# stecrotti/MPSKit.jl

Hardware: AMD Instinct MI355X
Metric: DMRG sweeps/sec + ddAC matvec achieved-TFLOP/s, Heisenberg L=100 D=1024 fp64 (higher is better)
Workload: dtype f64; 1 GPU; Heisenberg S=1/2 FiniteMPS L=100 D=1024 d=2 W=5 fp64, 1-site DMRG sweep (2L-2 site updates), fixed Krylov budget 8 matvecs/site; parallelism=single GPU

## Files before the change

mpskit.jl_amd/csrc/mpsk_cholqr.hip:

```cpp
#include <hip/hip_runtime.h>
#include <cmath>
#include <cstdio>
#include <cstdlib>
#include <cstring>
#include <string>
#include "mpsk_internal.h"

namespace mpsk {

constexpr int CB = 64;
constexpr double CQ_FIRSTORDER_MAX = 1.0e-7;

__global__ __launch_bounds__(256) void cq_pad_identity_kernel(double* __restrict__ G, int npad, int n) {
  const int64_t total = (int64_t)npad * npad;
  for (int64_t e = blockIdx.x * (int64_t)blockDim.x + threadIdx.x; e < total; e += (int64_t)gridDim.x * blockDim.x) {
    int r = (int)(e % npad), c = (int)(e / npad);
    if (r >= n || c >= n) G[e] = (r == c) ? 1.0 : 0.0;
  }
}

__global__ __launch_bounds__(256) void cq_shift_kernel(double* __restrict__ G, int npad, int n, double factor) {
  __shared__ double red[4];
  __shared__ double sh;
  double acc = 0.0;
  for (int i = threadIdx.x; i < n; i += 256) acc += G[i + (int64_t)i * npad];
  for (int off = 32; off > 0; off >>= 1) acc += __shfl_down(acc, off, 64);
  if ((threadIdx.x & 63) == 0) red[threadIdx.x >> 6] = acc;
  __syncthreads();
  if (threadIdx.x == 0) sh = factor * (red[0] + red[1] + red[2] + red[3]);
  __syncthreads();
  const double s = sh;
  for (int i = threadIdx.x; i < n; i += 256) G[i + (int64_t)i * npad] += s;
}

typedef double cq_d4 __attribute__((ext_vector_type(4)));

__device__ __forceinline__ double cq_readlane(double v, int lane) {
  int lo = __double2loint(v), hi = __double2hiint(v);
  lo = __builtin_amdgcn_readlane(lo, lane);
  hi = __builtin_amdgcn_readlane(hi, lane);
  return __hiloint2double(hi, lo);
}

__device__ __forceinline__ void piv_rsqrt(double x, double* rs_out, double* sq_out) {
  double r = __builtin_amdgcn_rsq(x);
  r = r * (1.5 - 0.5 * x * r * r);
  r = r * (1.5 - 0.5 * x * r * r);
  double s = x * r;
  s = s + 0.5 * r * (x - s * s);
  *rs_out = r;
  *sq_out = s;
}

constexpr int CQ_SL = 66;
constexpr size_t CQ_STEP_LDS = (size_t)3 * CB * CQ_SL * sizeof(double);

typedef double cq_d2 __attribute__((ext_vector_type(2)));
__device__ __forceinline__ void cq_fetch_tile(cq_d2 (&r)[8], const double* __restrict__ src, int npad, int tid) {
#pragma unroll
  for (int q = 0; q < 8; ++q) {
    const int v = tid + 256 * q, r2 = (v & 31) * 2, c = v >> 5;
    r[q] = *reinterpret_cast<const cq_d2*>(&src[r2 + (int64_t)c * npad]);
  }
}
__device__ __forceinline__ void cq_put_tile(double* __restrict__ dst, const cq_d2 (&r)[8], int tid) {
#pragma unroll
  for (int q = 0; q < 8; ++q) {
    const int v = tid + 256 * q, r2 = (v & 31) * 2, c = v >> 5;
    *reinterpret_cast<cq_d2*>(&dst[c * CQ_SL + r2]) = r[q];
  }
}

__device__ __forceinline__ void cq_prod(cq_d4 (&acc)[2][2], const double* __restrict__ tA, const double* __restrict__ tB,
                                        double sign, int wr, int wc, int fr, int fq) {
  for (int l0 = 0; l0 < CB; l0 += 4) {
    double af[2], bf[2];
#pragma unroll
    for (int ti = 0; ti < 2; ++ti) af[ti] = sign * tA[(32 * wr + 16 * ti + fr) * CQ_SL + l0 + fq];
#pragma unroll
    for (int tj = 0; tj < 2; ++tj) bf[tj] = tB[(32 * wc + 16 * tj + fr) * CQ_SL + l0 + fq];
#pragma unroll
    for (int ti = 0; ti < 2; ++ti)
#pragma unroll
      for (int tj = 0; tj < 2; ++tj)
        acc[ti][tj] = __builtin_amdgcn_mfma_f64_16x16x4f64(af[ti], bf[tj], acc[ti][tj], 0, 0, 0);
  }
}

constexpr int CQ_GS = 16;

__global__ __launch_bounds__(256) void cq_gram_reduce_kernel(const double* __restrict__ Gp, int npad, double* __restrict__ G) {
  const int64_t np2 = (int64_t)npad * npad;
  for (int64_t e = blockIdx.x * (int64_t)blockDim.x + threadIdx.x; e < np2; e += (int64_t)gridDim.x * blockDim.x) {
    const int r = (int)(e % npad), c = (int)(e / npad);
    if (r / CB > c / CB) continue;
    double acc = 0.0;
#pragma unroll
    for (int sp = 0; sp < CQ_GS; ++sp) acc += Gp[(int64_t)sp * np2 + e];
    G[e] = acc;
  }
}

__device__ __forceinline__ void cq_fetch_tile_g(cq_d2 (&r)[8], const double* __restrict__ src, int ld, int row0, int col0,
                                                int m, int n, int tid) {
#pragma unroll
  for (int q = 0; q < 8; ++q) {
    const int v = tid + 256 * q, r2 = (v & 31) * 2, c = v >> 5;
    const int gr = row0 + r2, gc = col0 + c;
    cq_d2 t = {0.0, 0.0};
    if (gc < n) {
      const double* p = src + gr + (int64_t)gc * ld;
      if (gr < m) t.x = p[0];
      if (gr + 1 < m) t.y = p[1];
    }
    r[q] = t;
  }
}
__device__ __forceinline__ void cq_put_tile_T(double* __restrict__ dst, const cq_d2 (&r)[8], int tid) {
#pragma unroll
  for (int q = 0; q < 8; ++q) {
    const int v = tid + 256 * q, r2 = (v & 31) * 2, c = v >> 5;
    dst[r2 * CQ_SL + c] = r[q].x;
    dst[(r2 + 1) * CQ_SL + c] = r[q].y;
  }
}

__global__ __launch_bounds__(256) void cq_step_kernel(double* __restrict__ G, double* __restrict__ R,
                                                      double* __restrict__ Rinv, int npad, int k,
                                                      int* __restrict__ flag, double* __restrict__ B, int m, int n,
                                                      int ldb, int trsm, double* __restrict__ Gp) {
  extern __shared__ __attribute__((aligned(16))) double cq_sm[];
  double* sM = cq_sm;
  double* sJ = cq_sm + CB * CQ_SL;
  double* sI = cq_sm + 2 * CB * CQ_SL;
  const int tid = threadIdx.x, lane = tid & 63, wave = tid >> 6;
  const int wr = wave >> 1, wc = wave & 1, fq = lane >> 4, fr = lane & 15;
  const int nb = npad / CB, kk = k - 1, nt = (nb - k > 0) ? nb - k : 0;
  const int ntrail = (k == 0) ? 1 : nt * (nt + 1) / 2;
  const int b = blockIdx.x;
  cq_d4 acc[2][2];
  if (trsm && b >= ntrail + nt) {
    const int mt = (m + CB - 1) / CB;
    int t = b - ntrail - nt;
    const int cQ = k - 2;
    const bool hasQ = (cQ >= 0 && cQ < nb);
    if (hasQ && t < mt) {
      const int row0 = t * CB, col0 = cQ * CB;
      cq_d2 t0[8], t1[8], t2[8];
      cq_fetch_tile(t2, Rinv + (int64_t)cQ * CB * (npad + 1), npad, tid);
      if (cQ > 0) {
        cq_fetch_tile_g(t0, B, ldb, row0, col0 - CB, m, n, tid);
        cq_fetch_tile(t1, R + (int64_t)(cQ - 1) * CB + (int64_t)cQ * CB * npad, npad, tid);
      }
#pragma unroll
      for (int ti = 0; ti < 2; ++ti)
#pragma unroll
        for (int tj = 0; tj < 2; ++tj)
#pragma unroll
          for (int rg = 0; rg < 4; ++rg) {
            const int gr = row0 + 32 * wr + 16 * ti + fq + 4 * rg, gc = col0 + 32 * wc + 16 * tj + fr;
            acc[ti][tj][rg] = (gr < m && gc < n) ? B[gr + (int64_t)gc * ldb] : 0.0;
          }
      if (cQ > 0) {
        cq_put_tile_T(sM, t0, tid);
        cq_put_tile(sJ, t1, tid);
        __syncthreads();
        cq_prod(acc, sM, sJ, -1.0, wr, wc, fr, fq);
        __syncthreads();
      }
#pragma unroll
      for (int ti = 0; ti < 2; ++ti)
#pragma unroll
        for (int tj = 0; tj < 2; ++tj)
#pragma unroll
          for (int rg = 0; rg < 4; ++rg)
            sI[(32 * wr + 16 * ti + fq + 4 * rg) * CQ_SL + 32 * wc + 16 * tj + fr] = acc[ti][tj][rg];
      cq_put_tile(sJ, t2, tid);
      __syncthreads();
#pragma unroll
      for (int ti = 0; ti < 2; ++ti)
#pragma unroll
        for (int tj = 0; tj < 2; ++tj) acc[ti][tj] = cq_d4{0.0, 0.0, 0.0, 0.0};
      cq_prod(acc, sI, sJ, 1.0, wr, wc, fr, fq);
#pragma unroll
      for (int ti = 0; ti < 2; ++ti)
#pragma unroll
        for (int tj = 0; tj < 2; ++tj)
#pragma unroll
          for (int rg = 0; rg < 4; ++rg) {
            const int gr = row0 + 32 * wr + 16 * ti + fq + 4 * rg, gc = col0 + 32 * wc + 16 * tj + fr;
            if (gr < m && gc < n) B[gr + (int64_t)gc * ldb] = acc[ti][tj][rg];
          }
      return;
    }
    if (hasQ) t -= mt;
    const int nU = (k - 3 >= 0 && nb - k + 1 > 0) ? (nb - k + 1) * mt : 0;
    if (t >= nU) {
      t -= nU;
      const int j = k - 3, i = t / CQ_GS, sp = t % CQ_GS;
      if (Gp == nullptr || j < 0 || j >= nb || i > j) return;
      const int chunk = (mt + CQ_GS - 1) / CQ_GS;
      const int r0 = sp * chunk, r1 = (r0 + chunk < mt) ? r0 + chunk : mt;
#pragma unroll
      for (int ti = 0; ti < 2; ++ti)
#pragma unroll
        for (int tj = 0; tj < 2; ++tj) acc[ti][tj] = cq_d4{0.0, 0.0, 0.0, 0.0};
      cq_d2 t0[8], t1[8];
      if (r0 < r1) {
        cq_fetch_tile_g(t0, B, ldb, r0 * CB, i * CB, m, n, tid);
        if (i != j) cq_fetch_tile_g(t1, B, ldb, r0 * CB, j * CB, m, n, tid);
      }
      for (int rt = r0; rt < r1; ++rt) {
        __syncthreads();
        cq_put_tile(sM, t0, tid);
        if (i != j) cq_put_tile(sJ, t1, tid); else cq_put_tile(sJ, t0, tid);
        __syncthreads();
        if (rt + 1 < r1) {
          cq_fetch_tile_g(t0, B, ldb, (rt + 1) * CB, i * CB, m, n, tid);
          if (i != j) cq_fetch_tile_g(t1, B, ldb, (rt + 1) * CB, j * CB, m, n, tid);
        }
        cq_prod(acc, sM, sJ, 1.0, wr, wc, fr, fq);
      }
      double* Gt = Gp + (int64_t)sp * npad * npad + (int64_t)i * CB + (int64_t)j * CB * npad;
#pragma unroll
      for (int ti = 0; ti < 2; ++ti)
#pragma unroll
        for (int tj = 0; tj < 2; ++tj)
#pragma unroll
          for (int rg = 0; rg < 4; ++rg)
            Gt[(32 * wr + 16 * ti + fq + 4 * rg) + (int64_t)(32 * wc + 16 * tj + fr) * npad] = acc[ti][tj][rg];
      return;
    }
    const int l = k - 3;
    const int j = l + 2 + t / mt, rt = t % mt;
    if (l < 0 || j >= nb) return;
    const int row0 = rt * CB, col0 = j * CB;
    cq_d2 t0[8], t1[8];
    cq_fetch_tile_g(t0, B, ldb, row0, l * CB, m, n, tid);
    cq_fetch_tile(t1, R + (int64_t)l * CB + (int64_t)j * CB * npad, npad, tid);
#pragma unroll
    for (int ti = 0; ti < 2; ++ti)
#pragma unroll
      for (int tj = 0; tj < 2; ++tj)
#pragma unroll
        for (int rg = 0; rg < 4; ++rg) {
          const int gr = row0 + 32 * wr + 16 * ti + fq + 4 * rg, gc = col0 + 32 * wc + 16 * tj + fr;
          acc[ti][tj][rg] = (gr < m && gc < n) ? B[gr + (int64_t)gc * ldb] : 0.0;
        }
    cq_put_tile_T(sM, t0, tid);
    cq_put_tile(sJ, t1, tid);
    __syncthreads();
    cq_prod(acc, sM, sJ, -1.0, wr, wc, fr, fq);
#pragma unroll
    for (int ti = 0; ti < 2; ++ti)
#pragma unroll
      for (int tj = 0; tj < 2; ++tj)
#pragma unroll
        for (int rg = 0; rg < 4; ++rg) {
          const int gr = row0 + 32 * wr + 16 * ti + fq + 4 * rg, gc = col0 + 32 * wc + 16 * tj + fr;
          if (gr < m && gc < n) B[gr + (int64_t)gc * ldb] = acc[ti][tj][rg];
        }
    return;
  }
  if (!trsm && k >= 2 && (k & 1) == 0 && b == ntrail + nt) {
    const int a = k - 2;
    cq_d2 t0[8], t1[8], t2[8];
    cq_fetch_tile(t0, Rinv + (int64_t)a * CB * (npad + 1), npad, tid);
    cq_fetch_tile(t1, R + (int64_t)a * CB + (int64_t)(a + 1) * CB * npad, npad, tid);
    cq_fetch_tile(t2, Rinv + (int64_t)(a + 1) * CB * (npad + 1), npad, tid);
#pragma unroll
    for (int q = 0; q < 8; ++q) {
      const int v = tid + 256 * q, r2 = (v & 31) * 2, c = v >> 5;
      sM[r2 * CQ_SL + c] = t0[q].x;
      sM[(r2 + 1) * CQ_SL + c] = t0[q].y;
    }
    cq_put_tile(sJ, t1, tid);
    __syncthreads();
#pragma unroll
    for (int ti = 0; ti < 2; ++ti)
#pragma unroll
      for (int tj = 0; tj < 2; ++tj) acc[ti][tj] = cq_d4{0.0, 0.0, 0.0, 0.0};
    cq_prod(acc, sM, sJ, 1.0, wr, wc, fr, fq);
    __syncthreads();
#pragma unroll
    for (int ti = 0; ti < 2; ++ti)
#pragma unroll
      for (int tj = 0; tj < 2; ++tj)
#pragma unroll
        for (int rg = 0; rg < 4; ++rg)
          sI[(32 * wr + 16 * ti + fq + 4 * rg) * CQ_SL + 32 * wc + 16 * tj + fr] = acc[ti][tj][rg];
    cq_put_tile(sJ, t2, tid);
    __syncthreads();
#pragma unroll
    for (int ti = 0; ti < 2; ++ti)
#pragma unroll
      for (int tj = 0; tj < 2; ++tj) acc[ti][tj] = cq_d4{0.0, 0.0, 0.0, 0.0};
    cq_prod(acc, sI, sJ, -1.0, wr, wc, fr, fq);
    double* Xb = Rinv + (int64_t)a * CB + (int64_t)(a + 1) * CB * npad;
#pragma unroll
    for (int ti = 0; ti < 2; ++ti)
#pragma unroll
      for (int tj = 0; tj < 2; ++tj)
#pragma unroll
        for (int rg = 0; rg < 4; ++rg)
          Xb[(32 * wr + 16 * ti + fq + 4 * rg) + (int64_t)(32 * wc + 16 * tj + fr) * npad] = acc[ti][tj][rg];
    return;
  }
  if (b >= ntrail) {
    const int j = k + (b - ntrail);
    cq_d2 t0[8], t1[8];
    cq_fetch_tile(t0, Rinv + (int64_t)kk * CB * (npad + 1), npad, tid);
    cq_fetch_tile(t1, G + (int64_t)kk * CB + (int64_t)j * CB * npad, npad, tid);
    cq_put_tile(sM, t0, tid);
    cq_put_tile(sJ, t1, tid);
    __syncthreads();
#pragma unroll
    for (int ti = 0; ti < 2; ++ti)
#pragma unroll
      for (int tj = 0; tj < 2; ++tj) acc[ti][tj] = cq_d4{0.0, 0.0, 0.0, 0.0};
    cq_prod(acc, sM, sJ, 1.0, wr, wc, fr, fq);
    double* Rb = R + (int64_t)kk * CB + (int64_t)j * CB * npad;
#pragma unroll
    for (int ti = 0; ti < 2; ++ti)
#pragma unroll
      for (int tj = 0; tj < 2; ++tj)
#pragma unroll
        for (int rg = 0; rg < 4; ++rg)
          Rb[(32 * wr + 16 * ti + fq + 4 * rg) + (int64_t)(32 * wc + 16 * tj + fr) * npad] = acc[ti][tj][rg];
    return;
  }
  int i = k, j = k;
  if (k > 0) {
    int ii = 0, rem = b;
    while (rem >= nt - ii) { rem -= nt - ii; ++ii; }
    i = k + ii; j = i + rem;
  }
  double* Gij = G + (int64_t)i * CB + (int64_t)j * CB * npad;
  cq_d2 t0[8], t1[8], t2[8];
  if (k > 0) {
    cq_fetch_tile(t0, Rinv + (int64_t)kk * CB * (npad + 1), npad, tid);
    cq_fetch_tile(t1, G + (int64_t)kk * CB + (int64_t)j * CB * npad, npad, tid);
    cq_fetch_tile(t2, G + (int64_t)kk * CB + (int64_t)i * CB * npad, npad, tid);
  }
#pragma unroll
  for (int ti = 0; ti < 2; ++ti)
#pragma unroll
    for (int tj = 0; tj < 2; ++tj)
#pragma unroll
      for (int rg = 0; rg < 4; ++rg)
        acc[ti][tj][rg] = Gij[(32 * wr + 16 * ti + fq + 4 * rg) + (int64_t)(32 * wc + 16 * tj + fr) * npad];
  if (k > 0) {
    cq_put_tile(sM, t0, tid);
    cq_put_tile(sJ, t1, tid);
    cq_put_tile(sI, t2, tid);
    __syncthreads();
    cq_d4 yj[2][2], yi[2][2];
#pragma unroll
    for (int ti = 0; ti < 2; ++ti)
#pragma unroll
      for (int tj = 0; tj < 2; ++tj) { yj[ti][tj] = cq_d4{0.0, 0.0, 0.0, 0.0}; yi[ti][tj] = cq_d4{0.0, 0.0, 0.0, 0.0}; }
    cq_prod(yj, sM, sJ, 1.0, wr, wc, fr, fq);
    if (i == j) {
#pragma unroll
      for (int ti = 0; ti < 2; ++ti)
#pragma unroll
        for (int tj = 0; tj < 2; ++tj) yi[ti][tj] = yj[ti][tj];
    } else {
      cq_prod(yi, sM, sI, 1.0, wr, wc, fr, fq);
    }
    __syncthreads();
#pragma unroll
    for (int ti = 0; ti < 2; ++ti)
#pragma unroll
      for (int tj = 0; tj < 2; ++tj)
#pragma unroll
        for (int rg = 0; rg < 4; ++rg) {
          const int o = (32 * wc + 16 * tj + fr) * CQ_SL + 32 * wr + 16 * ti + fq + 4 * rg;
          sJ[o] = yj[ti][tj][rg];
          sI[o] = yi[ti][tj][rg];
        }
    __syncthreads();
    cq_prod(acc, sI, sJ, -1.0, wr, wc, fr, fq);
  }
  if (b != 0) {
#pragma unroll
    for (int ti = 0; ti < 2; ++ti)
#pragma unroll
      for (int tj = 0; tj < 2; ++tj)
#pragma unroll
        for (int rg = 0; rg < 4; ++rg)
          Gij[(32 * wr + 16 * ti + fq + 4 * rg) + (int64_t)(32 * wc + 16 * tj + fr) * npad] = acc[ti][tj][rg];
    return;
  }
  __syncthreads();
  double (*P)[4][2 * CB] = reinterpret_cast<double (*)[4][2 * CB]>(cq_sm);
  cq_d4 accE[2][2];
#pragma unroll
  for (int ti = 0; ti < 2; ++ti)
#pragma unroll
    for (int tj = 0; tj < 2; ++tj)
#pragma unroll
      for (int rg = 0; rg < 4; ++rg)
        accE[ti][tj][rg] = ((32 * wr + 16 * ti + fq + 4 * rg) == (32 * wc + 16 * tj + fr)) ? 1.0 : 0.0;
  double* Rk = R + (int64_t)k * CB * (npad + 1);
  double* Xk = Rinv + (int64_t)k * CB * (npad + 1);
  int bad = 0;
  for (int rb = 0; rb < 2; ++rb)
#pragma unroll
  for (int ti = 0; ti < 2; ++ti)
#pragma unroll
  for (int q = 0; q < 4; ++q) {
    const int c = 8 * rb + 4 * ti + q;
    const int j0 = 4 * c;
    double (*Pb)[2 * CB] = P[c & 1];
    if (wr == rb) {
#pragma unroll
      for (int tj = 0; tj < 2; ++tj) {
        Pb[fq][32 * wc + 16 * tj + fr] = acc[ti][tj][q];
        Pb[fq][CB + 32 * wc + 16 * tj + fr] = accE[ti][tj][q];
      }
    }
    __syncthreads();
    if (wave == 0) {
      double p[4], e[4];
#pragma unroll
      for (int t = 0; t < 4; ++t) { p[t] = Pb[t][lane]; e[t] = Pb[t][CB + lane]; }
#pragma unroll
      for (int t = 0; t < 4; ++t) {
        const double piv = cq_readlane(p[t], j0 + t);
        const bool ok = (piv > 0.0) && (piv < 1.0e300);
        if (!ok) bad = 1;
        double rs_, sq_;
        piv_rsqrt(ok ? piv : 1.0, &rs_, &sq_);
        const double sq = ok ? sq_ : 1.0;
        const double rs = ok ? rs_ : 0.0;
        p[t] = (lane > j0 + t) ? p[t] * rs : (lane == j0 + t ? sq : 0.0);
        e[t] *= rs;
#pragma unroll
        for (int u = t + 1; u < 4; ++u) {
          const double r = cq_readlane(p[t], j0 + u);
          p[u] -= r * p[t];
          e[u] -= r * e[t];
        }
      }
#pragma unroll
      for (int t = 0; t < 4; ++t) {
        Pb[t][lane] = p[t];
        Pb[t][CB + lane] = e[t];
        Rk[(j0 + t) + (int64_t)lane * npad] = p[t];
        Xk[lane + (int64_t)(j0 + t) * npad] = e[t];
      }
    }
    __syncthreads();
    double af[2], bf[2], be[2];
#pragma unroll
    for (int t2 = 0; t2 < 2; ++t2) af[t2] = -Pb[fq][32 * wr + 16 * t2 + fr];
#pragma unroll
    for (int tj = 0; tj < 2; ++tj) { bf[tj] = Pb[fq][32 * wc + 16 * tj + fr]; be[tj] = Pb[fq][CB + 32 * wc + 16 * tj + fr]; }
#pragma unroll
    for (int t2 = 0; t2 < 2; ++t2)
#pragma unroll
      for (int tj = 0; tj < 2; ++tj) {
        acc[t2][tj] = __builtin_amdgcn_mfma_f64_16x16x4f64(af[t2], bf[tj], acc[t2][tj], 0, 0, 0);
        accE[t2][tj] = __builtin_amdgcn_mfma_f64_16x16x4f64(af[t2], be[tj], accE[t2][tj], 0, 0, 0);
      }
  }
  if (wave == 0 && lane == 0 && bad) atomicOr(flag, 1);
}

__global__ __launch_bounds__(256) void cq_cleanup_kernel(double* __restrict__ R, double* __restrict__ Rinv, int npad) {
  const int64_t total = (int64_t)npad * npad;
  for (int64_t e = blockIdx.x * (int64_t)blockDim.x + threadIdx.x; e < total; e += (int64_t)gridDim.x * blockDim.x) {
    int r = (int)(e % npad), c = (int)(e / npad);
    if (r / CB > c / CB) R[e] = 0.0;
    if (r / CB != c / CB && !(r / (2 * CB) == c / (2 * CB) && r / CB < c / CB)) Rinv[e] = 0.0;
  }
}

__global__ __launch_bounds__(256) void cq_check_identity_kernel(const double* __restrict__ G, int npad, int n,
                                                                double thresh, int* __restrict__ flag) {
  const int64_t total = (int64_t)n * n;
  int bad = 0;
  for (int64_t e = blockIdx.x * (int64_t)blockDim.x + threadIdx.x; e < total; e += (int64_t)gridDim.x * blockDim.x) {
    int r = (int)(e % n), c = (int)(e / n);
    if (r > c) continue;
    double v = G[r + (int64_t)c * npad] - (r == c ? 1.0 : 0.0);
    if (!(fabs(v) <= thresh)) bad = 1;
  }
  if (bad) atomicOr(flag, 2);
}

static bool cq_use_trsm(int m, int npad) {
  static const bool enabled = !(getenv("MPSK_CQ_TRSM") && atoi(getenv("MPSK_CQ_TRSM")) == 0);
  return enabled && (int64_t)(npad / CB) * ((m + CB - 1) / CB) <= 768;
}
static bool cq_use_gram(int m, int npad) {
  static const bool enabled = !(getenv("MPSK_CQ_GRAM") && atoi(getenv("MPSK_CQ_GRAM")) == 0);
  return enabled && cq_use_trsm(m, npad);
}

size_t cholqr_workspace_doubles(int m, int n) {
  int nb = (n + CB - 1) / CB, p2 = 1;
  while (p2 < nb) p2 <<= 1;
  size_t npad = (size_t)p2 * CB;
  return 5 * npad * npad + 2 * (size_t)m * n + 16 + (cq_use_gram(m, (int)npad) ? (size_t)CQ_GS * npad * npad : 0);
}

static GemmArgs cq_mk(const double* A, const double* B, double* C, int M, int N, int K, int64_t lda, int64_t ldb,
                      int64_t ldc, int tA, double alpha, double beta) {
  GemmArgs g;
  std::memset(&g, 0, sizeof(g));
  g.A = A; g.B = B; g.C = C; g.M = M; g.N = N; g.K = K; g.lda = lda; g.ldb = ldb; g.ldc = ldc;
  g.batch = 1; g.nseg = 1; g.alpha = alpha; g.beta = beta; g.transA = tA; g.transB = 0;
  return g;
}

static hipError_t cq_pass(int m, int n, int npad, const double* X, int ldx, double* Q, int ldq, double* Rp,
                          double* Rinv, double* T, bool shifted, bool check_identity, int* flag, hipStream_t s,
                          double shift_scale = 1.0, bool gram_ready = false, double* Gp_next = nullptr) {
  hipError_t e;
  double* Gw = T;
  GemmArgs g = cq_mk(X, X, Gw, n, n, m, ldx, ldx, npad, 1, 1.0, 0.0);
  g.upper_only = 1;
  if (!gram_ready && (e = gemm_f64(g, s)) != hipSuccess) return e;
  if (npad > n) hipLaunchKernelGGL(cq_pad_identity_kernel, dim3(512), dim3(256), 0, s, Gw, npad, n);
  if (check_identity) hipLaunchKernelGGL(cq_check_identity_kernel, dim3(256), dim3(256), 0, s, Gw, npad, n, 0.5, flag);
  if (shifted) {
    const double u = 1.1102230246251565e-16;
    const double factor = shift_scale * 11.0 * ((double)m * n + (double)n * (n + 1)) * u;
    hipLaunchKernelGGL(cq_shift_kernel, dim3(1), dim3(256), 0, s, Gw, npad, n, factor);
  }
  const int nb = npad / CB;
  static std::atomic<uint64_t> step_attr{0};
  if ((e = ensure_dyn_smem(step_attr, reinterpret_cast<const void*>(cq_step_kernel), CQ_STEP_LDS)) != hipSuccess) return e;
  const bool use_trsm = cq_use_trsm(m, npad);
  if (use_trsm) {
    if (X != Q) {
      if ((e = hipMemcpy2DAsync(Q, sizeof(double) * (size_t)ldq, X, sizeof(double) * (size_t)ldx, sizeof(double) * (size_t)m, n,
                                hipMemcpyDeviceToDevice, s)) != hipSuccess) return e;
    }
    const int mt = (m + CB - 1) / CB;
    for (int k = 0; k <= nb + (Gp_next ? 2 : 1); ++k) {
      const int nt = (nb - k > 0) ? nb - k : 0;
      int nwg = (k == 0) ? 1 : nt * (nt + 1) / 2 + nt;
      if (k - 2 >= 0 && k - 2 < nb) nwg += mt;
      if (k - 3 >= 0 && nb - k + 1 > 0) nwg += (nb - k + 1) * mt;
      if (Gp_next && k - 3 >= 0 && k - 3 < nb) nwg += (k - 2) * CQ_GS;
      if (nwg > 0)
        hipLaunchKernelGGL(cq_step_kernel, dim3(nwg), dim3(256), CQ_STEP_LDS, s, Gw, Rp, Rinv, npad, k, flag, Q, m, n, ldq, 1,
                           Gp_next);
    }
    hipLaunchKernelGGL(cq_cleanup_kernel, dim3(1024), dim3(256), 0, s, Rp, Rinv, npad);
    if (Gp_next) hipLaunchKernelGGL(cq_gram_reduce_kernel, dim3(1024), dim3(256), 0, s, Gp_next, npad, T);
    return hipGetLastError();
  }
  for (int k = 0; k <= nb; ++k) {
    const int nt = nb - k;
    const int pairwg = (k >= 2 && (k & 1) == 0) ? 1 : 0;
    const int nwg = (k == 0) ? 1 : nt * (nt + 1) / 2 + nt + pairwg;
    if (nwg > 0)
      hipLaunchKernelGGL(cq_step_kernel, dim3(nwg), dim3(256), CQ_STEP_LDS, s, Gw, Rp, Rinv, npad, k, flag, (double*)nullptr, 0, 0, 0, 0,
                         (double*)nullptr);
  }
  hipLaunchKernelGGL(cq_cleanup_kernel, dim3(1024), dim3(256), 0, s, Rp, Rinv, npad);
  for (int b = 2 * CB; b < npad; b <<= 1) {
    const int pairs = npad / (2 * b);
    const int64_t bs = (int64_t)2 * b * (npad + 1);
    const int64_t off12 = (int64_t)b * npad;
    const int64_t off22 = (int64_t)b * (npad + 1);
    g = cq_mk(Rp + off12, Rinv + off22, T + off12, b, b, b, npad, npad, npad, 0, 1.0, 0.0);
    g.batch = pairs; g.bsA = bs; g.bsB = bs; g.bsC = bs;
    if ((e = gemm_f64(g, s)) != hipSuccess) return e;
    g = cq_mk(Rinv, T + off12, Rinv + off12, b, b, b, npad, npad, npad, 0, -1.0, 0.0);
    g.batch = pairs; g.bsA = bs; g.bsB = bs; g.bsC = bs;
    if ((e = gemm_f64(g, s)) != hipSuccess) return e;
  }
  g = cq_mk(X, Rinv, Q, m, n, n, ldx, npad, ldq, 0, 1.0, 0.0);
  g.b_upper = 1;
  return gemm_f64(g, s);
}

__global__ __launch_bounds__(256) void cq_copy_upper_kernel(const double* __restrict__ Rp, int npad, int n,
                                                            double* __restrict__ R, int ldr) {
  const int64_t total = (int64_t)n * n;
  for (int64_t e = blockIdx.x * (int64_t)blockDim.x + threadIdx.x; e < total; e += (int64_t)gridDim.x * blockDim.x) {
    int r = (int)(e % n), c = (int)(e / n);
    R[r + (int64_t)c * ldr] = (r <= c) ? Rp[r + (int64_t)c * npad] : 0.0;
  }
}

__global__ __launch_bounds__(256) void cq_firstorder_kernel(const double* __restrict__ G, int npad, int n,
                                                            double* __restrict__ R3, double* __restrict__ Minv,
                                                            int* __restrict__ flag, double thr) {
  const int64_t total = (int64_t)npad * npad;
  int big = 0;
  for (int64_t e = blockIdx.x * (int64_t)blockDim.x + threadIdx.x; e < total; e += (int64_t)gridDim.x * blockDim.x) {
    int r = (int)(e % npad), c = (int)(e / npad);
    double u = 0.0, id = (r == c) ? 1.0 : 0.0;
    if (r < n && c < n && r <= c) {
      const double ev = G[e] - id;
      if (!(fabs(ev) <= 1.0e-7)) big = 1;
      u = (r < c) ? ev : 0.5 * ev;
    }
    R3[e] = id + u;
    Minv[e] = id - u;
  }
  if (big) atomicOr(flag, 4);
}

static hipError_t cq_pass_firstorder(int m, int n, int npad, const double* X, int ldx, double* Q, int ldq, double* Rp,
                                     double* Rinv, double* T, int* flag, hipStream_t s, bool gram_ready = false) {
  hipError_t e;
  GemmArgs g = cq_mk(X, X, T, n, n, m, ldx, ldx, npad, 1, 1.0, 0.0);
  g.upper_only = 1;
  if (!gram_ready && (e = gemm_f64(g, s)) != hipSuccess) return e;
  hipLaunchKernelGGL(cq_firstorder_kernel, dim3(1024), dim3(256), 0, s, T, npad, n, Rp, Rinv, flag, CQ_FIRSTORDER_MAX);
  g = cq_mk(X, Rinv, Q, m, n, n, ldx, npad, ldq, 0, 1.0, 0.0);
  g.b_upper = 1;
  return gemm_f64(g, s);
}

struct CqBufs { double *R1, *R2, *R3, *Rinv, *T, *Qa, *Qb, *Gp; int npad; };
static CqBufs cq_bufs(int m, int n, double* ws) {
  int nb = (n + CB - 1) / CB, p2 = 1;
  while (p2 < nb) p2 <<= 1;
  CqBufs b;
  b.npad = p2 * CB;
  const size_t np2 = (size_t)b.npad * b.npad;
  b.R1 = ws; b.R2 = b.R1 + np2; b.R3 = b.R2 + np2; b.Rinv = b.R3 + np2; b.T = b.Rinv + np2;
  b.Qa = b.T + np2; b.Qb = b.Qa + (size_t)m * n;
  b.Gp = cq_use_gram(m, b.npad) ? b.Qb + (((size_t)m * n + 1) & ~(size_t)1) : nullptr;
  return b;
}
static hipError_t cq_finish(const CqBufs& b, int n, double* R, int ldr, int* d_flag, int* flag_out, hipStream_t s) {
  hipError_t e;
  GemmArgs g = cq_mk(b.R2, b.R1, b.T, b.npad, b.npad, b.npad, b.npad, b.npad, b.npad, 0, 1.0, 0.0);
  g.a_upper = g.b_upper = g.upper_only = 1;
  if ((e = gemm_f64(g, s)) != hipSuccess) return e;
  g = cq_mk(b.R3, b.T, b.Rinv, b.npad, b.npad, b.npad, b.npad, b.npad, b.npad, 0, 1.0, 0.0);
  g.a_upper = g.b_upper = g.upper_only = 1;
  if ((e = gemm_f64(g, s)) != hipSuccess) return e;
  hipLaunchKernelGGL(cq_copy_upper_kernel, dim3(1024), dim3(256), 0, s, b.Rinv, b.npad, n, R, ldr);
  return hipMemcpyAsync(flag_out, d_flag, sizeof(int), hipMemcpyDeviceToHost, s);
}

static void cq_dbg_count(bool rep) {
  static long n = 0, r = 0;
  if (!getenv("MPSK_CQ_DEBUG")) return;
  ++n; if (rep) ++r;
  if (n % 100 == 0) fprintf(stderr, "[cholqr3] %ld factorizations, %ld repeated the third pass (thr %.1e)\n", n, r, CQ_FIRSTORDER_MAX);
}
hipError_t cholqr3_enqueue(int m, int n, const double* A, int lda, double* Q, int ldq, double* R, int ldr, double* ws,
                           int* d_flag, int* flag_out, hipStream_t s, double shift_scale) {
  const CqBufs b = cq_bufs(m, n, ws);
  hipError_t e;
  if ((e = hipMemsetAsync(d_flag, 0, sizeof(int), s)) != hipSuccess) return e;
  const bool gr = (b.Gp != nullptr);
  if ((e = cq_pass(m, n, b.npad, A, lda, b.Qa, m, b.R1, b.Rinv, b.T, true, false, d_flag, s, shift_scale, false, b.Gp)) != hipSuccess) return e;
  if ((e = cq_pass(m, n, b.npad, b.Qa, m, b.Qb, m, b.R2, b.Rinv, b.T, false, false, d_flag, s, 1.0, gr, b.Gp)) != hipSuccess) return e;
  if ((e = cq_pass_firstorder(m, n, b.npad, b.Qb, m, Q, ldq, b.R3, b.Rinv, b.T, d_flag, s, gr)) != hipSuccess) return e;
  return cq_finish(b, n, R, ldr, d_flag, flag_out, s);
}

hipError_t cholqr3_finalize(int m, int n, double* Q, int ldq, double* R, int ldr, double* ws, int* d_flag,
                            int* flag_out, hipStream_t s) {
  const CqBufs b = cq_bufs(m, n, ws);
  hipError_t e;
  if ((e = hipStreamSynchronize(s)) != hipSuccess) return e;
  cq_dbg_count(*flag_out == 4);
  if (*flag_out == 4) {
    if ((e = hipMemsetAsync(d_flag, 0, sizeof(int), s)) != hipSuccess) return e;
    if ((e = cq_pass(m, n, b.npad, b.Qb, m, Q, ldq, b.R3, b.Rinv, b.T, false, true, d_flag, s)) != hipSuccess) return e;
    if ((e = cq_finish(b, n, R, ldr, d_flag, flag_out, s)) != hipSuccess) return e;
    if ((e = hipStreamSynchronize(s)) != hipSuccess) return e;
  }
  return hipGetLastError();
}

__global__ __launch_bounds__(256) void cq_sumsq_kernel(const double* __restrict__ A, int lda, int m, int n,
                                                       double* __restrict__ out) {
  __shared__ double red[4];
  const int64_t total = (int64_t)m * n;
  double acc = 0.0;
  for (int64_t e = blockIdx.x * (int64_t)blockDim.x + threadIdx.x; e < total; e += (int64_t)gridDim.x * blockDim.x) {
    const double v = A[(e % m) + (e / m) * (int64_t)lda];
    acc += v * v;
  }
  for (int off = 32; off > 0; off >>= 1) acc += __shfl_down(acc, off, 64);
  if ((threadIdx.x & 63) == 0) red[threadIdx.x >> 6] = acc;
  __syncthreads();
  if (threadIdx.x == 0) out[1 + blockIdx.x] = red[0] + red[1] + red[2] + red[3];
}
__global__ __launch_bounds__(64) void cq_sumsq_final_kernel(double* __restrict__ out, int nblocks) {
  if (threadIdx.x == 0) {
    double acc = 0.0;
    for (int i = 0; i < nblocks; ++i) acc += out[1 + i];
    out[0] = acc;
  }
}
__global__ __launch_bounds__(256) void cq_perturb_kernel(const double* __restrict__ A, int lda, int m, int n,
                                                         double* __restrict__ X, int ldx, const double* __restrict__ sumsq) {
  const double delta = 1.1102230246251565e-16 * sqrt(sumsq[0] / (double)m);
  const int64_t total = (int64_t)m * n;
  for (int64_t e = blockIdx.x * (int64_t)blockDim.x + threadIdx.x; e < total; e += (int64_t)gridDim.x * blockDim.x) {
    const unsigned r = (unsigned)(e % m), c = (unsigned)(e / m);
    unsigned h = (r * 0x9E3779B1u) ^ (c * 0x85EBCA77u);
    h ^= h >> 15; h *= 0x2C1B3C6Du; h ^= h >> 12;
    X[r + (int64_t)c * ldx] = A[r + (int64_t)c * lda] + ((h & 1u) ? delta : -delta);
  }
}

hipError_t cholqr_robust(int m, int n, const double* A, int lda, double* Q, int ldq, double* R, int ldr, double* ws,
                         int* d_flag, int* flag_out, hipStream_t s) {
  const CqBufs b = cq_bufs(m, n, ws);
  const int npad = b.npad;
  hipError_t e;
  double* sumsq = b.T;
  if ((e = hipMemsetAsync(d_flag, 0, sizeof(int), s)) != hipSuccess) return e;
  hipLaunchKernelGGL(cq_sumsq_kernel, dim3(512), dim3(256), 0, s, A, lda, m, n, sumsq);
  hipLaunchKernelGGL(cq_sumsq_final_kernel, dim3(1), dim3(64), 0, s, sumsq, 512);
  hipLaunchKernelGGL(cq_perturb_kernel, dim3(1024), dim3(256), 0, s, A, lda, m, n, b.Qa, m, sumsq);
  double *acc = b.R1, *cur = b.R2, *tmp = b.R3;
  double *X = b.Qa, *Y = b.Qb;
  auto accumulate = [&]() -> hipError_t {
    GemmArgs g = cq_mk(cur, acc, tmp, npad, npad, npad, npad, npad, npad, 0, 1.0, 0.0);
    g.a_upper = g.b_upper = g.upper_only = 1;
    hipError_t ee = gemm_f64(g, s);
    double* t = acc; acc = tmp; tmp = t;
    return ee;
  };
  const double shift_rel = 11.0 * ((double)m * n + (double)n * (n + 1)) * 1.1102230246251565e-16;
  int nshift = (int)std::ceil(12.0 / (-0.5 * std::log10(shift_rel)));
  if (nshift < 3) nshift = 3;
  if (nshift > 6) nshift = 6;
  for (int p = 0; p < nshift + 1; ++p) {
    double* Rp = (p == 0) ? acc : cur;
    if ((e = cq_pass(m, n, npad, X, m, Y, m, Rp, b.Rinv, b.T, p < nshift, false, d_flag, s)) != hipSuccess) return e;
    if (p > 0 && (e = accumulate()) != hipSuccess) return e;
    double* t = X; X = Y; Y = t;
  }
  if ((e = cq_pass_firstorder(m, n, npad, X, m, Q, ldq, cur, b.Rinv, b.T, d_flag, s)) != hipSuccess) return e;
  if ((e = accumulate()) != hipSuccess) return e;
  hipLaunchKernelGGL(cq_copy_upper_kernel, dim3(1024), dim3(256), 0, s, acc, npad, n, R, ldr);
  if ((e = hipMemcpyAsync(flag_out, d_flag, sizeof(int), hipMemcpyDeviceToHost, s)) != hipSuccess) return e;
  if ((e = hipStreamSynchronize(s)) != hipSuccess) return e;
  if (*flag_out == 4) {
    { double* t = acc; acc = tmp; tmp = t; }
    if ((e = hipMemsetAsync(d_flag, 0, sizeof(int), s)) != hipSuccess) return e;
    if ((e = cq_pass(m, n, npad, X, m, Y, m, cur, b.Rinv, b.T, false, false, d_flag, s)) != hipSuccess) return e;
    if ((e = accumulate()) != hipSuccess) return e;
    if ((e = cq_pass_firstorder(m, n, npad, Y, m, Q, ldq, cur, b.Rinv, b.T, d_flag, s)) != hipSuccess) return e;
    if ((e = accumulate()) != hipSuccess) return e;
    hipLaunchKernelGGL(cq_copy_upper_kernel, dim3(1024), dim3(256), 0, s, acc, npad, n, R, ldr);
    if ((e = hipMemcpyAsync(flag_out, d_flag, sizeof(int), hipMemcpyDeviceToHost, s)) != hipSuccess) return e;
    if ((e = hipStreamSynchronize(s)) != hipSuccess) return e;
  }
  return hipGetLastError();
}

hipError_t cholqr1_orth(int m, int n, const double* X, int ldx, double* Q, int ldq, double* ws, int* d_flag, hipStream_t s,
                        double shift_scale) {
  const CqBufs b = cq_bufs(m, n, ws);
  hipError_t e;
  if ((e = hipMemsetAsync(d_flag, 0, sizeof(int), s)) != hipSuccess) return e;
  return cq_pass(m, n, b.npad, X, ldx, Q, ldq, b.R1, b.Rinv, b.T, true, false, d_flag, s, shift_scale);
}

hipError_t cholqr3(int m, int n, const double* A, int lda, double* Q, int ldq, double* R, int ldr, double* ws,
                   int* d_flag, int* flag_out, hipStream_t s, double shift_scale) {
  hipError_t e = cholqr3_enqueue(m, n, A, lda, Q, ldq, R, ldr, ws, d_flag, flag_out, s, shift_scale);
  if (e != hipSuccess) return e;
  return cholqr3_finalize(m, n, Q, ldq, R, ldr, ws, d_flag, flag_out, s);
}

}
```

Baseline: 1.166 sweeps/s.

## Fuse CholeskyQR diagonal-block factorization into head and close kernels, dropping one step launch

Result: no change. 1.177 sweeps/s (median of 6 runs) (+1.0%).

```diff
diff --git a/mpskit.jl_amd/csrc/mpsk_cholqr.hip b/mpskit.jl_amd/csrc/mpsk_cholqr.hip
--- a/mpskit.jl_amd/csrc/mpsk_cholqr.hip
+++ b/mpskit.jl_amd/csrc/mpsk_cholqr.hip
@@ -17,20 +17,6 @@
     int r = (int)(e % npad), c = (int)(e / npad);
     if (r >= n || c >= n) G[e] = (r == c) ? 1.0 : 0.0;
   }
-}
-
-__global__ __launch_bounds__(256) void cq_shift_kernel(double* __restrict__ G, int npad, int n, double factor) {
-  __shared__ double red[4];
-  __shared__ double sh;
-  double acc = 0.0;
-  for (int i = threadIdx.x; i < n; i += 256) acc += G[i + (int64_t)i * npad];
-  for (int off = 32; off > 0; off >>= 1) acc += __shfl_down(acc, off, 64);
-  if ((threadIdx.x & 63) == 0) red[threadIdx.x >> 6] = acc;
-  __syncthreads();
-  if (threadIdx.x == 0) sh = factor * (red[0] + red[1] + red[2] + red[3]);
-  __syncthreads();
-  const double s = sh;
-  for (int i = threadIdx.x; i < n; i += 256) G[i + (int64_t)i * npad] += s;
 }
 
 typedef double cq_d4 __attribute__((ext_vector_type(4)));
@@ -52,6 +38,116 @@
   *sq_out = s;
 }
 
+constexpr size_t CQ_FACTOR_LDS = (size_t)2 * 4 * 2 * CB * sizeof(double);
+__device__ __forceinline__ void cq_factor_diag(cq_d4 (&acc)[2][2], double* __restrict__ lds, double* __restrict__ Rk,
+                                               double* __restrict__ Xk, int npad, int* __restrict__ flag) {
+  const int tid = threadIdx.x, lane = tid & 63, wave = tid >> 6;
+  const int wr = wave >> 1, wc = wave & 1, fq = lane >> 4, fr = lane & 15;
+  __syncthreads();
+  double (*P)[4][2 * CB] = reinterpret_cast<double (*)[4][2 * CB]>(lds);
+  cq_d4 accE[2][2];
+#pragma unroll
+  for (int ti = 0; ti < 2; ++ti)
+#pragma unroll
+    for (int tj = 0; tj < 2; ++tj)
+#pragma unroll
+      for (int rg = 0; rg < 4; ++rg)
+        accE[ti][tj][rg] = ((32 * wr + 16 * ti + fq + 4 * rg) == (32 * wc + 16 * tj + fr)) ? 1.0 : 0.0;
+  int bad = 0;
+  for (int rb = 0; rb < 2; ++rb)
+#pragma unroll
+  for (int ti = 0; ti < 2; ++ti)
+#pragma unroll
+  for (int q = 0; q < 4; ++q) {
+    const int c = 8 * rb + 4 * ti + q;
+    const int j0 = 4 * c;
+    double (*Pb)[2 * CB] = P[c & 1];
+    if (wr == rb) {
+#pragma unroll
+      for (int tj = 0; tj < 2; ++tj) {
+        Pb[fq][32 * wc + 16 * tj + fr] = acc[ti][tj][q];
+        Pb[fq][CB + 32 * wc + 16 * tj + fr] = accE[ti][tj][q];
+      }
+    }
+    __syncthreads();
+    if (wave == 0) {
+      double p[4], e[4];
+#pragma unroll
+      for (int t = 0; t < 4; ++t) { p[t] = Pb[t][lane]; e[t] = Pb[t][CB + lane]; }
+#pragma unroll
+      for (int t = 0; t < 4; ++t) {
+        const double piv = cq_readlane(p[t], j0 + t);
+        const bool ok = (piv > 0.0) && (piv < 1.0e300);
+        if (!ok) bad = 1;
+        double rs_, sq_;
+        piv_rsqrt(ok ? piv : 1.0, &rs_, &sq_);
+        const double sq = ok ? sq_ : 1.0;
+        const double rs = ok ? rs_ : 0.0;
+        p[t] = (lane > j0 + t) ? p[t] * rs : (lane == j0 + t ? sq : 0.0);
+        e[t] *= rs;
+#pragma unroll
+        for (int u = t + 1; u < 4; ++u) {
+          const double r = cq_readlane(p[t], j0 + u);
+          p[u] -= r * p[t];
+          e[u] -= r * e[t];
+        }
+      }
+#pragma unroll
+      for (int t = 0; t < 4; ++t) {
+        Pb[t][lane] = p[t];
+        Pb[t][CB + lane] = e[t];
+        Rk[(j0 + t) + (int64_t)lane * npad] = p[t];
+        Xk[lane + (int64_t)(j0 + t) * npad] = e[t];
+      }
+    }
+    __syncthreads();
+    double af[2], bf[2], be[2];
+#pragma unroll
+    for (int t2 = 0; t2 < 2; ++t2) af[t2] = -Pb[fq][32 * wr + 16 * t2 + fr];
+#pragma unroll
+    for (int tj = 0; tj < 2; ++tj) { bf[tj] = Pb[fq][32 * wc + 16 * tj + fr]; be[tj] = Pb[fq][CB + 32 * wc + 16 * tj + fr]; }
+#pragma unroll
+    for (int t2 = 0; t2 < 2; ++t2)
+#pragma unroll
+      for (int tj = 0; tj < 2; ++tj) {
+        acc[t2][tj] = __builtin_amdgcn_mfma_f64_16x16x4f64(af[t2], bf[tj], acc[t2][tj], 0, 0, 0);
+        accE[t2][tj] = __builtin_amdgcn_mfma_f64_16x16x4f64(af[t2], be[tj], accE[t2][tj], 0, 0, 0);
+      }
+  }
+  if (wave == 0 && lane == 0 && bad) atomicOr(flag, 1);
+}
+
+__global__ __launch_bounds__(256) void cq_head_kernel(double* G, int npad, int n, double factor, int shifted,
+                                                      double* __restrict__ R, double* __restrict__ Rinv,
+                                                      int* __restrict__ flag) {
+  __shared__ double red[4];
+  __shared__ double sh;
+  __shared__ __attribute__((aligned(16))) double fac_sm[CQ_FACTOR_LDS / sizeof(double)];
+  if (shifted) {
+    double tr = 0.0;
+    for (int i = threadIdx.x; i < n; i += 256) tr += G[i + (int64_t)i * npad];
+    for (int off = 32; off > 0; off >>= 1) tr += __shfl_down(tr, off, 64);
+    if ((threadIdx.x & 63) == 0) red[threadIdx.x >> 6] = tr;
+    __syncthreads();
+    if (threadIdx.x == 0) sh = factor * (red[0] + red[1] + red[2] + red[3]);
+    __syncthreads();
+    const double s = sh;
+    for (int i = threadIdx.x; i < n; i += 256) G[i + (int64_t)i * npad] += s;
+    __syncthreads();
+  }
+  const int tid = threadIdx.x, lane = tid & 63, wave = tid >> 6;
+  const int wr = wave >> 1, wc = wave & 1, fq = lane >> 4, fr = lane & 15;
+  cq_d4 acc[2][2];
+#pragma unroll
+  for (int ti = 0; ti < 2; ++ti)
+#pragma unroll
+    for (int tj = 0; tj < 2; ++tj)
+#pragma unroll
+      for (int rg = 0; rg < 4; ++rg)
+        acc[ti][tj][rg] = G[(32 * wr + 16 * ti + fq + 4 * rg) + (int64_t)(32 * wc + 16 * tj + fr) * npad];
+  cq_factor_diag(acc, fac_sm, R, Rinv, npad, flag);
+}
+
 constexpr int CQ_SL = 66;
 constexpr size_t CQ_STEP_LDS = (size_t)3 * CB * CQ_SL * sizeof(double);
 
@@ -89,14 +185,55 @@
 
 constexpr int CQ_GS = 16;
 
-__global__ __launch_bounds__(256) void cq_gram_reduce_kernel(const double* __restrict__ Gp, int npad, double* __restrict__ G) {
+__global__ __launch_bounds__(256) void cq_close_kernel(double* __restrict__ R, double* __restrict__ Rinv, int npad, int n,
+                                                       const double* __restrict__ Gp, double* G,
+                                                       double* __restrict__ Rnext, int* __restrict__ flag) {
+  __shared__ __attribute__((aligned(16))) double fac_sm[CQ_FACTOR_LDS / sizeof(double)];
   const int64_t np2 = (int64_t)npad * npad;
-  for (int64_t e = blockIdx.x * (int64_t)blockDim.x + threadIdx.x; e < np2; e += (int64_t)gridDim.x * blockDim.x) {
+  const int tid = threadIdx.x;
+  if (Rnext != nullptr && blockIdx.x == 0) {
+    cq_d2 sum[8];
+#pragma unroll
+    for (int q = 0; q < 8; ++q) sum[q] = cq_d2{0.0, 0.0};
+#pragma unroll
+    for (int sp = 0; sp < CQ_GS; ++sp) {
+      cq_d2 t[8];
+      cq_fetch_tile(t, Gp + (int64_t)sp * np2, npad, tid);
+#pragma unroll
+      for (int q = 0; q < 8; ++q) sum[q] += t[q];
+    }
+#pragma unroll
+    for (int q = 0; q < 8; ++q) {
+      const int v = tid + 256 * q, r2 = (v & 31) * 2, c = v >> 5;
+      if (r2 >= n || c >= n) sum[q].x = (r2 == c) ? 1.0 : 0.0;
+      if (r2 + 1 >= n || c >= n) sum[q].y = (r2 + 1 == c) ? 1.0 : 0.0;
+      *reinterpret_cast<cq_d2*>(&G[r2 + (int64_t)c * npad]) = sum[q];
+    }
+    __syncthreads();
+    const int lane = tid & 63, wave = tid >> 6;
+    const int wr = wave >> 1, wc = wave & 1, fq = lane >> 4, fr = lane & 15;
+    cq_d4 acc[2][2];
+#pragma unroll
+    for (int ti = 0; ti < 2; ++ti)
+#pragma unroll
+      for (int tj = 0; tj < 2; ++tj)
+#pragma unroll
+        for (int rg = 0; rg < 4; ++rg)
+          acc[ti][tj][rg] = G[(32 * wr + 16 * ti + fq + 4 * rg) + (int64_t)(32 * wc + 16 * tj + fr) * npad];
+    cq_factor_diag(acc, fac_sm, Rnext, Rinv, npad, flag);
+    return;
+  }
+  const int lead = (Rnext != nullptr) ? 1 : 0;
+  const int64_t stride = (int64_t)(gridDim.x - lead) * blockDim.x;
+  for (int64_t e = (blockIdx.x - lead) * (int64_t)blockDim.x + tid; e < np2; e += stride) {
     const int r = (int)(e % npad), c = (int)(e / npad);
-    if (r / CB > c / CB) continue;
+    if (r / CB > c / CB) R[e] = 0.0;
+    if (r / CB != c / CB && !(r / (2 * CB) == c / (2 * CB) && r / CB < c / CB)) Rinv[e] = 0.0;
+    if (Gp == nullptr || r / CB > c / CB || (lead && r < CB && c < CB)) continue;
     double acc = 0.0;
 #pragma unroll
     for (int sp = 0; sp < CQ_GS; ++sp) acc += Gp[(int64_t)sp * np2 + e];
+    if (r >= n || c >= n) acc = (r == c) ? 1.0 : 0.0;
     G[e] = acc;
   }
 }
@@ -136,13 +273,13 @@
   const int tid = threadIdx.x, lane = tid & 63, wave = tid >> 6;
   const int wr = wave >> 1, wc = wave & 1, fq = lane >> 4, fr = lane & 15;
   const int nb = npad / CB, kk = k - 1, nt = (nb - k > 0) ? nb - k : 0;
-  const int ntrail = (k == 0) ? 1 : nt * (nt + 1) / 2;
+  const int ntrail = nt * (nt + 1) / 2;
   const int b = blockIdx.x;
   cq_d4 acc[2][2];
   if (trsm && b >= ntrail + nt) {
     const int mt = (m + CB - 1) / CB;
     int t = b - ntrail - nt;
-    const int cQ = k - 2;
+    const int cQ = k - 1;
     const bool hasQ = (cQ >= 0 && cQ < nb);
     if (hasQ && t < mt) {
       const int row0 = t * CB, col0 = cQ * CB;
@@ -194,10 +331,10 @@
       return;
     }
     if (hasQ) t -= mt;
-    const int nU = (k - 3 >= 0 && nb - k + 1 > 0) ? (nb - k + 1) * mt : 0;
+    const int nU = (k - 2 >= 0 && nb - k > 0) ? (nb - k) * mt : 0;
     if (t >= nU) {
       t -= nU;
-      const int j = k - 3, i = t / CQ_GS, sp = t % CQ_GS;
+      const int j = k - 2, i = t / CQ_GS, sp = t % CQ_GS;
       if (Gp == nullptr || j < 0 || j >= nb || i > j) return;
       const int chunk = (mt + CQ_GS - 1) / CQ_GS;
       const int r0 = sp * chunk, r1 = (r0 + chunk < mt) ? r0 + chunk : mt;
@@ -231,7 +368,7 @@
             Gt[(32 * wr + 16 * ti + fq + 4 * rg) + (int64_t)(32 * wc + 16 * tj + fr) * npad] = acc[ti][tj][rg];
       return;
     }
-    const int l = k - 3;
+    const int l = k - 2;
     const int j = l + 2 + t / mt, rt = t % mt;
     if (l < 0 || j >= nb) return;
     const int row0 = rt * CB, col0 = j * CB;
@@ -329,19 +466,14 @@
           Rb[(32 * wr + 16 * ti + fq + 4 * rg) + (int64_t)(32 * wc + 16 * tj + fr) * npad] = acc[ti][tj][rg];
     return;
   }
-  int i = k, j = k;
-  if (k > 0) {
-    int ii = 0, rem = b;
-    while (rem >= nt - ii) { rem -= nt - ii; ++ii; }
-    i = k + ii; j = i + rem;
-  }
+  int ii = 0, rem = b;
+  while (rem >= nt - ii) { rem -= nt - ii; ++ii; }
+  const int i = k + ii, j = i + rem;
   double* Gij = G + (int64_t)i * CB + (int64_t)j * CB * npad;
   cq_d2 t0[8], t1[8], t2[8];
-  if (k > 0) {
-    cq_fetch_tile(t0, Rinv + (int64_t)kk * CB * (npad + 1), npad, tid);
-    cq_fetch_tile(t1, G + (int64_t)kk * CB + (int64_t)j * CB * npad, npad, tid);
-    cq_fetch_tile(t2, G + (int64_t)kk * CB + (int64_t)i * CB * npad, npad, tid);
-  }
+  cq_fetch_tile(t0, Rinv + (int64_t)kk * CB * (npad + 1), npad, tid);
+  cq_fetch_tile(t1, G + (int64_t)kk * CB + (int64_t)j * CB * npad, npad, tid);
+  cq_fetch_tile(t2, G + (int64_t)kk * CB + (int64_t)i * CB * npad, npad, tid);
 #pragma unroll
   for (int ti = 0; ti < 2; ++ti)
 #pragma unroll
@@ -349,39 +481,37 @@
 #pragma unroll
       for (int rg = 0; rg < 4; ++rg)
         acc[ti][tj][rg] = Gij[(32 * wr + 16 * ti + fq + 4 * rg) + (int64_t)(32 * wc + 16 * tj + fr) * npad];
-  if (k > 0) {
-    cq_put_tile(sM, t0, tid);
-    cq_put_tile(sJ, t1, tid);
-    cq_put_tile(sI, t2, tid);
-    __syncthreads();
-    cq_d4 yj[2][2], yi[2][2];
-#pragma unroll
-    for (int ti = 0; ti < 2; ++ti)
-#pragma unroll
-      for (int tj = 0; tj < 2; ++tj) { yj[ti][tj] = cq_d4{0.0, 0.0, 0.0, 0.0}; yi[ti][tj] = cq_d4{0.0, 0.0, 0.0, 0.0}; }
-    cq_prod(yj, sM, sJ, 1.0, wr, wc, fr, fq);
-    if (i == j) {
-#pragma unroll
-      for (int ti = 0; ti < 2; ++ti)
-#pragma unroll
-        for (int tj = 0; tj < 2; ++tj) yi[ti][tj] = yj[ti][tj];
-    } else {
-      cq_prod(yi, sM, sI, 1.0, wr, wc, fr, fq);
-    }
-    __syncthreads();
-#pragma unroll
-    for (int ti = 0; ti < 2; ++ti)
-#pragma unroll
-      for (int tj = 0; tj < 2; ++tj)
-#pragma unroll
-        for (int rg = 0; rg < 4; ++rg) {
-          const int o = (32 * wc + 16 * tj + fr) * CQ_SL + 32 * wr + 16 * ti + fq + 4 * rg;
-          sJ[o] = yj[ti][tj][rg];
-          sI[o] = yi[ti][tj][rg];
-        }
-    __syncthreads();
-    cq_prod(acc, sI, sJ, -1.0, wr, wc, fr, fq);
-  }
+  cq_put_tile(sM, t0, tid);
+  cq_put_tile(sJ, t1, tid);
+  cq_put_tile(sI, t2, tid);
+  __syncthreads();
+  cq_d4 yj[2][2], yi[2][2];
+#pragma unroll
+  for (int ti = 0; ti < 2; ++ti)
+#pragma unroll
+    for (int tj = 0; tj < 2; ++tj) { yj[ti][tj] = cq_d4{0.0, 0.0, 0.0, 0.0}; yi[ti][tj] = cq_d4{0.0, 0.0, 0.0, 0.0}; }
+  cq_prod(yj, sM, sJ, 1.0, wr, wc, fr, fq);
+  if (i == j) {
+#pragma unroll
+    for (int ti = 0; ti < 2; ++ti)
+#pragma unroll
+      for (int tj = 0; tj < 2; ++tj) yi[ti][tj] = yj[ti][tj];
+  } else {
+    cq_prod(yi, sM, sI, 1.0, wr, wc, fr, fq);
+  }
+  __syncthreads();
+#pragma unroll
+  for (int ti = 0; ti < 2; ++ti)
+#pragma unroll
+    for (int tj = 0; tj < 2; ++tj)
+#pragma unroll
+      for (int rg = 0; rg < 4; ++rg) {
+        const int o = (32 * wc + 16 * tj + fr) * CQ_SL + 32 * wr + 16 * ti + fq + 4 * rg;
+        sJ[o] = yj[ti][tj][rg];
+        sI[o] = yi[ti][tj][rg];
+      }
+  __syncthreads();
+  cq_prod(acc, sI, sJ, -1.0, wr, wc, fr, fq);
   if (b != 0) {
 #pragma unroll
     for (int ti = 0; ti < 2; ++ti)
@@ -392,89 +522,7 @@
           Gij[(32 * wr + 16 * ti + fq + 4 * rg) + (int64_t)(32 * wc + 16 * tj + fr) * npad] = acc[ti][tj][rg];
     return;
   }
-  __syncthreads();
-  double (*P)[4][2 * CB] = reinterpret_cast<double (*)[4][2 * CB]>(cq_sm);
-  cq_d4 accE[2][2];
-#pragma unroll
-  for (int ti = 0; ti < 2; ++ti)
-#pragma unroll
-    for (int tj = 0; tj < 2; ++tj)
-#pragma unroll
-      for (int rg = 0; rg < 4; ++rg)
-        accE[ti][tj][rg] = ((32 * wr + 16 * ti + fq + 4 * rg) == (32 * wc + 16 * tj + fr)) ? 1.0 : 0.0;
-  double* Rk = R + (int64_t)k * CB * (npad + 1);
-  double* Xk = Rinv + (int64_t)k * CB * (npad + 1);
-  int bad = 0;
-  for (int rb = 0; rb < 2; ++rb)
-#pragma unroll
-  for (int ti = 0; ti < 2; ++ti)
-#pragma unroll
-  for (int q = 0; q < 4; ++q) {
-    const int c = 8 * rb + 4 * ti + q;
-    const int j0 = 4 * c;
-    double (*Pb)[2 * CB] = P[c & 1];
-    if (wr == rb) {
-#pragma unroll
-      for (int tj = 0; tj < 2; ++tj) {
-        Pb[fq][32 * wc + 16 * tj + fr] = acc[ti][tj][q];
-        Pb[fq][CB + 32 * wc + 16 * tj + fr] = accE[ti][tj][q];
-      }
-    }
-    __syncthreads();
-    if (wave == 0) {
-      double p[4], e[4];
-#pragma unroll
-      for (int t = 0; t < 4; ++t) { p[t] = Pb[t][lane]; e[t] = Pb[t][CB + lane]; }
-#pragma unroll
-      for (int t = 0; t < 4; ++t) {
-        const double piv = cq_readlane(p[t], j0 + t);
-        const bool ok = (piv > 0.0) && (piv < 1.0e300);
-        if (!ok) bad = 1;
-        double rs_, sq_;
-        piv_rsqrt(ok ? piv : 1.0, &rs_, &sq_);
-        const double sq = ok ? sq_ : 1.0;
-        const double rs = ok ? rs_ : 0.0;
-        p[t] = (lane > j0 + t) ? p[t] * rs : (lane == j0 + t ? sq : 0.0);
-        e[t] *= rs;
-#pragma unroll
-        for (int u = t + 1; u < 4; ++u) {
-          const double r = cq_readlane(p[t], j0 + u);
-          p[u] -= r * p[t];
-          e[u] -= r * e[t];
-        }
-      }
-#pragma unroll
-      for (int t = 0; t < 4; ++t) {
-        Pb[t][lane] = p[t];
-        Pb[t][CB + lane] = e[t];
-        Rk[(j0 + t) + (int64_t)lane * npad] = p[t];
-        Xk[lane + (int64_t)(j0 + t) * npad] = e[t];
-      }
-    }
-    __syncthreads();
-    double af[2], bf[2], be[2];
-#pragma unroll
-    for (int t2 = 0; t2 < 2; ++t2) af[t2] = -Pb[fq][32 * wr + 16 * t2 + fr];
-#pragma unroll
-    for (int tj = 0; tj < 2; ++tj) { bf[tj] = Pb[fq][32 * wc + 16 * tj + fr]; be[tj] = Pb[fq][CB + 32 * wc + 16 * tj + fr]; }
-#pragma unroll
-    for (int t2 = 0; t2 < 2; ++t2)
-#pragma unroll
-      for (int tj = 0; tj < 2; ++tj) {
-        acc[t2][tj] = __builtin_amdgcn_mfma_f64_16x16x4f64(af[t2], bf[tj], acc[t2][tj], 0, 0, 0);
-        accE[t2][tj] = __builtin_amdgcn_mfma_f64_16x16x4f64(af[t2], be[tj], accE[t2][tj], 0, 0, 0);
-      }
-  }
-  if (wave == 0 && lane == 0 && bad) atomicOr(flag, 1);
-}
-
-__global__ __launch_bounds__(256) void cq_cleanup_kernel(double* __restrict__ R, double* __restrict__ Rinv, int npad) {
-  const int64_t total = (int64_t)npad * npad;
-  for (int64_t e = blockIdx.x * (int64_t)blockDim.x + threadIdx.x; e < total; e += (int64_t)gridDim.x * blockDim.x) {
-    int r = (int)(e % npad), c = (int)(e / npad);
-    if (r / CB > c / CB) R[e] = 0.0;
-    if (r / CB != c / CB && !(r / (2 * CB) == c / (2 * CB) && r / CB < c / CB)) Rinv[e] = 0.0;
-  }
+  cq_factor_diag(acc, cq_sm, R + (int64_t)k * CB * (npad + 1), Rinv + (int64_t)k * CB * (npad + 1), npad, flag);
 }
 
 __global__ __launch_bounds__(256) void cq_check_identity_kernel(const double* __restrict__ G, int npad, int n,
@@ -517,18 +565,21 @@
 
 static hipError_t cq_pass(int m, int n, int npad, const double* X, int ldx, double* Q, int ldq, double* Rp,
                           double* Rinv, double* T, bool shifted, bool check_identity, int* flag, hipStream_t s,
-                          double shift_scale = 1.0, bool gram_ready = false, double* Gp_next = nullptr) {
+                          double shift_scale = 1.0, bool gram_ready = false, double* Gp_next = nullptr,
+                          double* Rp_next = nullptr) {
   hipError_t e;
   double* Gw = T;
-  GemmArgs g = cq_mk(X, X, Gw, n, n, m, ldx, ldx, npad, 1, 1.0, 0.0);
-  g.upper_only = 1;
-  if (!gram_ready && (e = gemm_f64(g, s)) != hipSuccess) return e;
-  if (npad > n) hipLaunchKernelGGL(cq_pad_identity_kernel, dim3(512), dim3(256), 0, s, Gw, npad, n);
-  if (check_identity) hipLaunchKernelGGL(cq_check_identity_kernel, dim3(256), dim3(256), 0, s, Gw, npad, n, 0.5, flag);
-  if (shifted) {
+  if (gram_ready && (shifted || check_identity)) return hipErrorInvalidValue;
+  if (Rp_next && !Gp_next) return hipErrorInvalidValue;
+  if (!gram_ready) {
+    GemmArgs g = cq_mk(X, X, Gw, n, n, m, ldx, ldx, npad, 1, 1.0, 0.0);
+    g.upper_only = 1;
+    if ((e = gemm_f64(g, s)) != hipSuccess) return e;
+    if (npad > n) hipLaunchKernelGGL(cq_pad_identity_kernel, dim3(512), dim3(256), 0, s, Gw, npad, n);
+    if (check_identity) hipLaunchKernelGGL(cq_check_identity_kernel, dim3(256), dim3(256), 0, s, Gw, npad, n, 0.5, flag);
     const double u = 1.1102230246251565e-16;
     const double factor = shift_scale * 11.0 * ((double)m * n + (double)n * (n + 1)) * u;
-    hipLaunchKernelGGL(cq_shift_kernel, dim3(1), dim3(256), 0, s, Gw, npad, n, factor);
+    hipLaunchKernelGGL(cq_head_kernel, dim3(1), dim3(256), 0, s, Gw, npad, n, factor, shifted ? 1 : 0, Rp, Rinv, flag);
   }
   const int nb = npad / CB;
   static std::atomic<uint64_t> step_attr{0};
@@ -540,29 +591,32 @@
                                 hipMemcpyDeviceToDevice, s)) != hipSuccess) return e;
     }
     const int mt = (m + CB - 1) / CB;
-    for (int k = 0; k <= nb + (Gp_next ? 2 : 1); ++k) {
+    for (int k = 1; k <= nb + (Gp_next ? 1 : 0); ++k) {
       const int nt = (nb - k > 0) ? nb - k : 0;
-      int nwg = (k == 0) ? 1 : nt * (nt + 1) / 2 + nt;
-      if (k - 2 >= 0 && k - 2 < nb) nwg += mt;
-      if (k - 3 >= 0 && nb - k + 1 > 0) nwg += (nb - k + 1) * mt;
-      if (Gp_next && k - 3 >= 0 && k - 3 < nb) nwg += (k - 2) * CQ_GS;
+      int nwg = nt * (nt + 1) / 2 + nt;
+      if (k - 1 < nb) nwg += mt;
+      if (k - 2 >= 0 && nb - k > 0) nwg += (nb - k) * mt;
+      if (Gp_next && k - 2 >= 0 && k - 2 < nb) nwg += (k - 1) * CQ_GS;
       if (nwg > 0)
         hipLaunchKernelGGL(cq_step_kernel, dim3(nwg), dim3(256), CQ_STEP_LDS, s, Gw, Rp, Rinv, npad, k, flag, Q, m, n, ldq, 1,
                            Gp_next);
     }
-    hipLaunchKernelGGL(cq_cleanup_kernel, dim3(1024), dim3(256), 0, s, Rp, Rinv, npad);
-    if (Gp_next) hipLaunchKernelGGL(cq_gram_reduce_kernel, dim3(1024), dim3(256), 0, s, Gp_next, npad, T);
+    hipLaunchKernelGGL(cq_close_kernel, dim3(1024 + (Rp_next ? 1 : 0)), dim3(256), 0, s, Rp, Rinv, npad, n,
+                       (const double*)Gp_next, T, Rp_next, flag);
     return hipGetLastError();
   }
-  for (int k = 0; k <= nb; ++k) {
+  if (Gp_next) return hipErrorInvalidValue;
+  for (int k = 1; k <= nb; ++k) {
     const int nt = nb - k;
     const int pairwg = (k >= 2 && (k & 1) == 0) ? 1 : 0;
-    const int nwg = (k == 0) ? 1 : nt * (nt + 1) / 2 + nt + pairwg;
+    const int nwg = nt * (nt + 1) / 2 + nt + pairwg;
     if (nwg > 0)
       hipLaunchKernelGGL(cq_step_kernel, dim3(nwg), dim3(256), CQ_STEP_LDS, s, Gw, Rp, Rinv, npad, k, flag, (double*)nullptr, 0, 0, 0, 0,
                          (double*)nullptr);
   }
-  hipLaunchKernelGGL(cq_cleanup_kernel, dim3(1024), dim3(256), 0, s, Rp, Rinv, npad);
+  hipLaunchKernelGGL(cq_close_kernel, dim3(1024), dim3(256), 0, s, Rp, Rinv, npad, n, (const double*)nullptr, (double*)nullptr,
+                     (double*)nullptr, flag);
+  GemmArgs g;
   for (int b = 2 * CB; b < npad; b <<= 1) {
     const int pairs = npad / (2 * b);
     const int64_t bs = (int64_t)2 * b * (npad + 1);
@@ -656,7 +710,8 @@
   hipError_t e;
   if ((e = hipMemsetAsync(d_flag, 0, sizeof(int), s)) != hipSuccess) return e;
   const bool gr = (b.Gp != nullptr);
-  if ((e = cq_pass(m, n, b.npad, A, lda, b.Qa, m, b.R1, b.Rinv, b.T, true, false, d_flag, s, shift_scale, false, b.Gp)) != hipSuccess) return e;
+  if ((e = cq_pass(m, n, b.npad, A, lda, b.Qa, m, b.R1, b.Rinv, b.T, true, false, d_flag, s, shift_scale, false, b.Gp,
+                   gr ? b.R2 : nullptr)) != hipSuccess) return e;
   if ((e = cq_pass(m, n, b.npad, b.Qa, m, b.Qb, m, b.R2, b.Rinv, b.T, false, false, d_flag, s, 1.0, gr, b.Gp)) != hipSuccess) return e;
   if ((e = cq_pass_firstorder(m, n, b.npad, b.Qb, m, Q, ldq, b.R3, b.Rinv, b.T, d_flag, s, gr)) != hipSuccess) return e;
   return cq_finish(b, n, R, ldr, d_flag, flag_out, s);
```
